# near/near-light-client

Measured on AMD Instinct MI355X. Metric: Sync/Verify proofs/sec at 1/2/4/8 MI355X + achieved HBM GB/s vs roofline, higher is better.
Workload: dtype u64 (Goldilocks field, integer)

## Files before the change

near-light-client_amd/csrc/gl32.hpp:

```cpp
#pragma once
#include "gl.hpp"
#include "poseidon_blocks.inc"

namespace gl32 {

struct F {
    uint32_t lo, hi;
};

__device__ __forceinline__ F from_u64(uint64_t x) { return F{(uint32_t)x, (uint32_t)(x >> 32)}; }
__device__ __forceinline__ uint64_t to_u64(F x) { return ((uint64_t)x.hi << 32) | x.lo; }

__device__ __forceinline__ F add_w2_eps(uint64_t base, uint32_t w2) {
    uint64_t r;
    uint32_t t;
    asm("v_mad_u64_u32 %[r], vcc, %[w2], -1, %[base]\n\t"
        "v_cndmask_b32_e64 %[t], 0, -1, vcc\n\t"
        "v_mad_u64_u32 %[r], vcc, %[t], 1, %[r]"
        : [r] "=&v"(r), [t] "=&v"(t)
        : [w2] "v"(w2), [base] "v"(base)
        : "vcc");
    return from_u64(r);
}

__device__ __forceinline__ F reduce128(uint32_t w0, uint32_t w1, uint32_t w2, uint32_t w3) {
    uint32_t r0, r1, t0;
    asm("v_sub_co_u32 %[r0], vcc, %[w0], %[w3]\n\t"
        "v_subbrev_co_u32 %[r1], vcc, 0, %[w1], vcc\n\t"
        "v_cndmask_b32_e64 %[t0], 0, -1, vcc\n\t"
        "v_sub_co_u32 %[r0], vcc, %[r0], %[t0]\n\t"
        "v_subbrev_co_u32 %[r1], vcc, 0, %[r1], vcc"
        : [r0] "=&v"(r0), [r1] "=&v"(r1), [t0] "=&v"(t0)
        : [w0] "v"(w0), [w1] "v"(w1), [w3] "v"(w3)
        : "vcc");
    return add_w2_eps(((uint64_t)r1 << 32) | r0, w2);
}

__device__ __forceinline__ uint64_t mad_u64_one(uint32_t a, uint64_t c);

__device__ __forceinline__ F mul(F a, F b) {
#ifdef NLX_GL32_MUL_CARRY_CHAINS
    uint64_t t = (uint64_t)a.lo * b.lo;
    uint64_t m = (uint64_t)a.lo * b.hi;
    uint64_t x = (uint64_t)a.hi * b.hi;
    uint64_t mid;
    uint32_t x1;
    asm("v_mad_u64_u32 %[mid], vcc, %[ah], %[bl], %[m]\n\t"
        "v_addc_co_u32 %[x1], vcc, 0, %[xh], vcc"
        : [mid] "=&v"(mid), [x1] "=v"(x1)
        : [ah] "v"(a.hi), [bl] "v"(b.lo), [m] "v"(m), [xh] "v"((uint32_t)(x >> 32))
        : "vcc");
    uint32_t r0, r1, w1, w2, w3, t0;
    asm("v_add_co_u32 %[w1], vcc, %[th], %[m0]\n\t"
        "v_addc_co_u32 %[w2], vcc, %[x0], %[m1], vcc\n\t"
        "v_addc_co_u32 %[w3], vcc, 0, %[x1], vcc\n\t"
        "v_sub_co_u32 %[r0], vcc, %[w0], %[w3]\n\t"
        "v_subbrev_co_u32 %[r1], vcc, 0, %[w1], vcc\n\t"
        "v_cndmask_b32_e64 %[t0], 0, -1, vcc\n\t"
        "v_sub_co_u32 %[r0], vcc, %[r0], %[t0]\n\t"
        "v_subbrev_co_u32 %[r1], vcc, 0, %[r1], vcc"
        : [r0] "=&v"(r0), [r1] "=&v"(r1), [w1] "=&v"(w1), [w2] "=&v"(w2), [w3] "=&v"(w3), [t0] "=&v"(t0)
        : [w0] "v"((uint32_t)t), [th] "v"((uint32_t)(t >> 32)), [m0] "v"((uint32_t)mid), [x0] "v"((uint32_t)x),
          [m1] "v"((uint32_t)(mid >> 32)), [x1] "v"(x1)
        : "vcc");
    return add_w2_eps(((uint64_t)r1 << 32) | r0, w2);
#else
    const uint64_t p0 = (uint64_t)a.lo * b.lo;
    const uint64_t p1 = (uint64_t)a.lo * b.hi + (p0 >> 32);
    const uint64_t p2 = (uint64_t)a.hi * b.lo + (uint32_t)p1;
    uint64_t p3 = (uint64_t)a.hi * b.hi + (p1 >> 32);
    p3 = mad_u64_one((uint32_t)(p2 >> 32), p3);
    return reduce128((uint32_t)p0, (uint32_t)p2, (uint32_t)p3, (uint32_t)(p3 >> 32));
#endif
}

__device__ __forceinline__ F add_const(F a, uint64_t c) {
    F r;
    uint32_t t;
    asm("v_add_co_u32 %[r0], vcc, %[a0], %[c0]\n\t"
        "v_addc_co_u32 %[r1], vcc, %[a1], %[c1], vcc\n\t"
        "v_cndmask_b32_e64 %[t], 0, -1, vcc\n\t"
        "v_add_co_u32 %[r0], vcc, %[r0], %[t]\n\t"
        "v_addc_co_u32 %[r1], vcc, 0, %[r1], vcc"
        : [r0] "=&v"(r.lo), [r1] "=&v"(r.hi), [t] "=&v"(t)
        : [a0] "v"(a.lo), [a1] "v"(a.hi), [c0] "s"((uint32_t)c), [c1] "v"((uint32_t)(c >> 32))
        : "vcc");
    return r;
}

__device__ __forceinline__ F add_const_v(F a, uint64_t c) {
    F r;
    uint32_t t;
    asm("v_add_co_u32 %[r0], vcc, %[a0], %[c0]\n\t"
        "v_addc_co_u32 %[r1], vcc, %[a1], %[c1], vcc\n\t"
        "v_cndmask_b32_e64 %[t], 0, -1, vcc\n\t"
        "v_add_co_u32 %[r0], vcc, %[r0], %[t]\n\t"
        "v_addc_co_u32 %[r1], vcc, 0, %[r1], vcc"
        : [r0] "=&v"(r.lo), [r1] "=&v"(r.hi), [t] "=&v"(t)
        : [a0] "v"(a.lo), [a1] "v"(a.hi), [c0] "v"((uint32_t)c), [c1] "v"((uint32_t)(c >> 32))
        : "vcc");
    return r;
}

__device__ __forceinline__ F sbox7(F x) {
    F x2 = mul(x, x);
    F x4 = mul(x2, x2);
    F x3 = mul(x, x2);
    return mul(x3, x4);
}

__device__ __forceinline__ F fold_acc(uint64_t al, uint64_t ah) {
    uint64_t t;
    asm("v_mad_u64_u32 %[t], vcc, %[ah1], -1, %[al]" : [t] "=&v"(t) : [ah1] "v"((uint32_t)(ah >> 32)), [al] "v"(al) : "vcc");
    uint32_t r1, m;
    asm("v_add_co_u32 %[r1], vcc, %[t1], %[ah0]\n\t"
        "v_cndmask_b32_e64 %[m], 0, -1, vcc"
        : [r1] "=v"(r1), [m] "=v"(m)
        : [t1] "v"((uint32_t)(t >> 32)), [ah0] "v"((uint32_t)ah)
        : "vcc");
    uint64_t r;
    asm("v_mad_u64_u32 %[r], vcc, %[m], 1, %[base]" : [r] "=&v"(r) : [m] "v"(m), [base] "v"(((uint64_t)r1 << 32) | (uint32_t)t) : "vcc");
    return from_u64(r);
}

__device__ __forceinline__ void mds_layer(F (&s)[12], const uint64_t* __restrict__ rc_next = nullptr) {
    constexpr uint32_t C[12] = {17, 15, 41, 16, 2, 28, 13, 13, 39, 18, 34, 20};
    F o[12];
#pragma unroll
    for (int r = 0; r < 12; r++) {
        uint64_t al = 0, ah = 0;
        if (rc_next) {
            const uint64_t c = rc_next[r];
            al = (uint32_t)c;
            ah = c >> 32;
        }
#pragma unroll
        for (int i = 0; i < 12; i++) {
            al += (uint64_t)s[(i + r) % 12].lo * C[i];
            ah += (uint64_t)s[(i + r) % 12].hi * C[i];
        }
        if (r == 0) {
            al += (uint64_t)s[0].lo * 8u;
            ah += (uint64_t)s[0].hi * 8u;
        }
        o[r] = fold_acc(al, ah);
    }
#pragma unroll
    for (int i = 0; i < 12; i++) s[i] = o[i];
}


typedef int i32x4_t __attribute__((ext_vector_type(4)));
typedef int i32x16_t __attribute__((ext_vector_type(16)));

__device__ __forceinline__ void keep_whole(const i32x16_t& d) { asm volatile("" : : "v"(d)); }

__device__ __forceinline__ i32x4_t mds_a_fragment(uint32_t lane = threadIdx.x & 63) {
    constexpr int C[12] = {17, 15, 41, 16, 2, 28, 13, 13, 39, 18, 34, 20};
    const uint32_t rho = lane & 31, h = lane >> 5;
    const uint32_t g = (rho >> 2) & 1, r = (rho & 3) + 4 * (rho >> 3);
    uint32_t w[4] = {0, 0, 0, 0};
    if (h == g && rho < 24) {
#pragma unroll
        for (int j = 0; j < 12; j++) {
            uint32_t m = 0;
#pragma unroll
            for (int rr = 0; rr < 12; rr++)
                if ((uint32_t)rr == r) m = (uint32_t)C[(j - rr + 12) % 12] + ((rr == 0 && j == 0) ? 8u : 0u);
            w[j >> 2] |= m << (8 * (j & 3));
        }
        w[3] = r == 0 ? 0x00F88080u : 0x00008080u;
    }
    i32x4_t a;
    a.x = (int)w[0]; a.y = (int)w[1]; a.z = (int)w[2]; a.w = (int)w[3];
    return a;
}
constexpr uint32_t MDS_B_BIAS_SLOTS = 0x00808080u;

__device__ __forceinline__ void transpose_bytes4(uint32_t x0, uint32_t x1, uint32_t x2, uint32_t x3, uint32_t (&p)[4]) {
    const uint32_t t01l = __builtin_amdgcn_perm(x1, x0, 0x05010400u), t01h = __builtin_amdgcn_perm(x1, x0, 0x07030602u);
    const uint32_t t23l = __builtin_amdgcn_perm(x3, x2, 0x05010400u), t23h = __builtin_amdgcn_perm(x3, x2, 0x07030602u);
    p[0] = __builtin_amdgcn_perm(t23l, t01l, 0x05040100u);
    p[1] = __builtin_amdgcn_perm(t23l, t01l, 0x07060302u);
    p[2] = __builtin_amdgcn_perm(t23h, t01h, 0x05040100u);
    p[3] = __builtin_amdgcn_perm(t23h, t01h, 0x07060302u);
}
__device__ __forceinline__ uint64_t mad_u64(uint32_t a, uint32_t b, uint64_t c) {
    uint64_t r, sink;
    asm("v_mad_u64_u32 %0, %1, %2, %3, %4" : "=v"(r), "=s"(sink) : "v"(a), "v"(b), "v"(c));
    return r;
}
__device__ __forceinline__ uint64_t mad_u64_sc(uint32_t a, uint32_t b, uint64_t c_uniform) {
    uint64_t r, sink;
    asm("v_mad_u64_u32 %0, %1, %2, %3, %4" : "=v"(r), "=s"(sink) : "v"(a), "v"(b), "s"(c_uniform));
    return r;
}
__device__ __forceinline__ uint64_t mad_u64_one(uint32_t a, uint64_t c) {
    uint64_t r, sink;
    asm("v_mad_u64_u32 %0, %1, %2, 1, %3" : "=v"(r), "=s"(sink) : "v"(a), "v"(c));
    return r;
}
__device__ __forceinline__ F fold_pair(uint64_t t, uint32_t yh, uint32_t k16) {
    uint64_t z, u, sink, sink2;
    asm("v_mad_u64_u32 %0, %1, %2, %3, 0" : "=v"(z), "=s"(sink) : "v"(yh), "v"(k16));
    asm("v_mad_u64_u32 %0, %1, %2, -1, %3" : "=v"(u), "=s"(sink2) : "v"((uint32_t)(z >> 32)), "v"(t));
    uint32_t r1, m;
    asm("v_add_co_u32 %0, vcc, %2, %3\n\t"
        "v_cndmask_b32_e64 %1, 0, -1, vcc"
        : "=v"(r1), "=v"(m)
        : "v"((uint32_t)(u >> 32)), "v"((uint32_t)z)
        : "vcc");
    return from_u64(mad_u64_one(m, ((uint64_t)r1 << 32) | (uint32_t)u));
}

template <int RC>
__device__ __forceinline__ void mds_layer_mfma(F (&s)[12], const i32x4_t a, const uint64_t* __restrict__ rcb) {
    uint32_t k16 = 65536u, bw = MDS_B_BIAS_SLOTS;
    asm("" : "+v"(k16));
    asm("" : "+v"(bw));
    i32x16_t zero;
#pragma unroll
    for (int i = 0; i < 16; i++) zero[i] = 0;
    uint32_t x[2][12], y[2][12];
#pragma unroll
    for (int half = 0; half < 2; half++) {
        uint32_t pl[4][3];
#pragma unroll
        for (int q = 0; q < 3; q++) {
            uint32_t p[4];
            if (half == 0)
                transpose_bytes4(s[4 * q].lo ^ 0x80808080u, s[4 * q + 1].lo ^ 0x80808080u, s[4 * q + 2].lo ^ 0x80808080u,
                                 s[4 * q + 3].lo ^ 0x80808080u, p);
            else
                transpose_bytes4(s[4 * q].hi ^ 0x80808080u, s[4 * q + 1].hi ^ 0x80808080u, s[4 * q + 2].hi ^ 0x80808080u,
                                 s[4 * q + 3].hi ^ 0x80808080u, p);
#pragma unroll
            for (int b = 0; b < 4; b++) pl[b][q] = p[b];
        }
        i32x16_t d[4];
#pragma unroll
        for (int b = 0; b < 4; b++) {
            i32x4_t bf;
            bf.x = (int)pl[b][0]; bf.y = (int)pl[b][1]; bf.z = (int)pl[b][2]; bf.w = (int)bw;
            d[b] = __builtin_amdgcn_mfma_i32_32x32x32_i8(a, bf, zero, 0, 0, 0);
        }
#pragma unroll
        for (int b = 0; b < 4; b++) keep_whole(d[b]);
#pragma unroll
        for (int r = 0; r < 12; r++) {
            x[half][r] = ((uint32_t)d[1][r] << 8) + (uint32_t)d[0][r];
            y[half][r] = ((uint32_t)d[3][r] << 8) + (uint32_t)d[2][r];
        }
        __builtin_amdgcn_sched_barrier(0);
    }
#pragma unroll
    for (int r = 0; r < 12; r++) {
        if (RC == 2 || (RC == 1 && r == 0)) {
            const uint64_t al = mad_u64_one(x[0][r], mad_u64_sc(y[0][r], k16, rcb[r]));
            const uint64_t ah = mad_u64_one(x[1][r], mad_u64_sc(y[1][r], k16, rcb[12 + r]));
            s[r] = fold_acc(al, ah);
        } else {
            const uint64_t t = mad_u64(y[0][r], k16, ((uint64_t)x[1][r] << 32) | x[0][r]);
            s[r] = fold_pair(t, y[1][r], k16);
        }
    }
}

struct BlockOperands {
    i32x4_t a[3];
    i32x16_t seed;
};

template <int G>
__device__ __forceinline__ uint64_t mad_u64_imm(uint32_t a, uint64_t c) {
    uint64_t r, sink;
    asm("v_mad_u64_u32 %0, %1, %2, %3, %4" : "=v"(r), "=s"(sink) : "v"(a), "n"(G), "v"(c));
    return r;
}
__device__ __forceinline__ F fold_pair_x(uint64_t t, uint32_t yh, uint32_t x2, uint32_t k16) {
    uint64_t z, u, sink, sink2;
    asm("v_mad_u64_u32 %0, %1, %2, %3, 0" : "=v"(z), "=s"(sink) : "v"(yh), "v"(k16));
    const uint32_t e = (uint32_t)(z >> 32) + x2;
    asm("v_mad_u64_u32 %0, %1, %2, -1, %3" : "=v"(u), "=s"(sink2) : "v"(e), "v"(t));
    uint32_t r1, m;
    asm("v_add_co_u32 %0, vcc, %2, %3\n\t"
        "v_cndmask_b32_e64 %1, 0, -1, vcc"
        : "=v"(r1), "=v"(m)
        : "v"((uint32_t)(u >> 32)), "v"((uint32_t)z)
        : "vcc");
    return from_u64(mad_u64_one(m, ((uint64_t)r1 << 32) | (uint32_t)u));
}
__device__ __forceinline__ uint64_t mad_u64_sm(uint32_t a, uint32_t m_uniform, uint64_t c) {
    uint64_t r, sink;
    asm("v_mad_u64_u32 %0, %1, %2, %3, %4" : "=v"(r), "=s"(sink) : "v"(a), "s"(m_uniform), "v"(c));
    return r;
}
template <typename RHO>
__device__ __forceinline__ void dot12(const F (&z)[12], const RHO& rho, uint64_t klo, uint64_t khi, uint64_t& al, uint64_t& ah) {
    al = klo;
    ah = khi;
#pragma unroll
    for (int j = 0; j < 12; j++) {
        al = mad_u64_sm(z[j].lo, rho.v[j], al);
        ah = mad_u64_sm(z[j].hi, rho.v[j], ah);
    }
}
struct BlockRho1 { static constexpr uint32_t v[12] = NLX_POSEIDON_BLOCK_RHO1_INIT; };
struct BlockRho2 { static constexpr uint32_t v[12] = NLX_POSEIDON_BLOCK_RHO2_INIT; };

struct BlockSboxes {
    __device__ __forceinline__ F first(F s0) const { return sbox7(s0); }
    __device__ __forceinline__ F inner(int, F w) const { return sbox7(w); }
    __device__ __forceinline__ void before_matrix_pass() const {}
};

template <int GAMMA21, class Sboxes = BlockSboxes>
__device__ __forceinline__ void partial_block3(F (&s)[12], const BlockOperands& op, const uint64_t* __restrict__ kap,
                                               Sboxes sb = Sboxes{}) {
    uint32_t k16 = 65536u;
    asm("" : "+v"(k16));
    s[0] = sb.first(s[0]);
    uint64_t al, ah;
    dot12(s, BlockRho1{}, kap[2], kap[3], al, ah);
    const F u1 = sb.inner(1, fold_acc(al, ah));
    dot12(s, BlockRho2{}, kap[4], kap[5], al, ah);
    al = mad_u64_imm<GAMMA21>(u1.lo, al);
    ah = mad_u64_imm<GAMMA21>(u1.hi, ah);
    const F u2 = sb.inner(2, fold_acc(al, ah));
    sb.before_matrix_pass();
    uint32_t pl[8][3];
#pragma unroll
    for (int half = 0; half < 2; half++)
#pragma unroll
        for (int q = 0; q < 3; q++) {
            uint32_t p[4];
            if (half == 0)
                transpose_bytes4(s[4 * q].lo ^ 0x80808080u, s[4 * q + 1].lo ^ 0x80808080u, s[4 * q + 2].lo ^ 0x80808080u,
                                 s[4 * q + 3].lo ^ 0x80808080u, p);
            else
                transpose_bytes4(s[4 * q].hi ^ 0x80808080u, s[4 * q + 1].hi ^ 0x80808080u, s[4 * q + 2].hi ^ 0x80808080u,
                                 s[4 * q + 3].hi ^ 0x80808080u, p);
#pragma unroll
            for (int b = 0; b < 4; b++) pl[4 * half + b][q] = p[b];
        }
    uint32_t w3[8];
    {
        const uint32_t a1l = u1.lo ^ 0x80808080u, a1h = u1.hi ^ 0x80808080u, a2l = u2.lo ^ 0x80808080u, a2h = u2.hi ^ 0x80808080u;
        w3[0] = __builtin_amdgcn_perm(a2l, a1l, 0x00000400u); w3[1] = __builtin_amdgcn_perm(a2l, a1l, 0x00000501u);
        w3[2] = __builtin_amdgcn_perm(a2l, a1l, 0x00000602u); w3[3] = __builtin_amdgcn_perm(a2l, a1l, 0x00000703u);
        w3[4] = __builtin_amdgcn_perm(a2h, a1h, 0x00000400u); w3[5] = __builtin_amdgcn_perm(a2h, a1h, 0x00000501u);
        w3[6] = __builtin_amdgcn_perm(a2h, a1h, 0x00000602u); w3[7] = __builtin_amdgcn_perm(a2h, a1h, 0x00000703u);
    }
    uint32_t x0[12], y0[12], y1[12];
    uint64_t tt[12];
    uint64_t ah0 = 0;
    auto chain = [&](int q) {
        i32x16_t d = op.seed;
#pragma unroll
        for (int p = 0; p < 3; p++)
            if (q - p >= 0 && q - p <= 7) {
                i32x4_t bf;
                bf.x = (int)pl[q - p][0]; bf.y = (int)pl[q - p][1]; bf.z = (int)pl[q - p][2]; bf.w = (int)w3[q - p];
                d = __builtin_amdgcn_mfma_i32_32x32x32_i8(op.a[p], bf, d, 0, 0, 0);
            }
        return d;
    };
#pragma unroll
    for (int pr = 0; pr < 5; pr++) {
        i32x16_t d[2];
        d[0] = chain(2 * pr);
        d[1] = chain(2 * pr + 1);
        keep_whole(d[0]);
        keep_whole(d[1]);
#pragma unroll
        for (int r = 0; r < 12; r++) {
            uint32_t x = ((uint32_t)d[1][r] << 8) + (uint32_t)d[0][r];
            asm("" : "+v"(x));
            if (pr == 0) x0[r] = x;
            if (pr == 1) {
                y0[r] = x;
                if (r == 0) tt[0] = mad_u64_one(x0[0], mad_u64_sc(x, k16, kap[0]));
            }
            if (pr == 2) {
                if (r == 0) ah0 = x;
                else tt[r] = mad_u64(y0[r], k16, ((uint64_t)x << 32) | x0[r]);
            }
            if (pr == 3) {
                y1[r] = x;
                if (r == 0) ah0 = mad_u64_one((uint32_t)ah0, mad_u64_sc(x, k16, kap[1]));
            }
            if (pr == 4) {
                if (r == 0) s[0] = fold_acc(tt[0], ah0 + ((uint64_t)x << 32));
                else s[r] = fold_pair_x(tt[r], y1[r], x, k16);
            }
        }
#ifndef NLX_PB_NO_BARRIER
        __builtin_amdgcn_sched_barrier(0);
#endif
    }
}

}
```

near-light-client_amd/csrc/hash_kernels.hip:

```cpp
#include <hip/hip_runtime.h>
#include "poseidon.hpp"
#include "launch.hpp"

namespace nlx {

__global__ __launch_bounds__(256, 4) void k_permute_batch(uint64_t* __restrict__ states, size_t n) {
    const size_t t_raw = (size_t)blockIdx.x * blockDim.x + threadIdx.x;
    const bool live = t_raw < n;
    const size_t t = live ? t_raw : n - 1;
    uint64_t s[12];
    const ulonglong2* src = reinterpret_cast<const ulonglong2*>(states + t * 12);
#pragma unroll
    for (int i = 0; i < 6; i++) {
        ulonglong2 v = src[i];
        s[2 * i] = v.x;
        s[2 * i + 1] = v.y;
    }
    poseidon::permute(s);
    if (!live) return;
    ulonglong2* dst = reinterpret_cast<ulonglong2*>(states + t * 12);
#pragma unroll
    for (int i = 0; i < 6; i++) dst[i] = make_ulonglong2(s[2 * i], s[2 * i + 1]);
}

__device__ __forceinline__ void store_digest(uint64_t* __restrict__ out, size_t idx, const uint64_t (&s)[12]) {
    ulonglong2* dst = reinterpret_cast<ulonglong2*>(out + idx * 4);
    dst[0] = make_ulonglong2(gl::canon(s[0]), gl::canon(s[1]));
    dst[1] = make_ulonglong2(gl::canon(s[2]), gl::canon(s[3]));
}

__global__ __launch_bounds__(256, 4) void k_hash_leaves_rowmajor(const uint64_t* __restrict__ rows, uint32_t row_len,
                                                              size_t n_rows, uint64_t* __restrict__ digests) {
    const size_t row_raw = (size_t)blockIdx.x * blockDim.x + threadIdx.x;
    const bool live = row_raw < n_rows;
    const size_t row = live ? row_raw : n_rows - 1;
    uint64_t s[12];
#pragma unroll
    for (int i = 0; i < 12; i++) s[i] = 0;
    const uint64_t* p = rows + row * (size_t)row_len;
    if (row_len <= 4) {
        for (uint32_t c = 0; c < row_len; c++) {
            uint64_t v = p[c];
            if (c == 0) s[0] = v; else if (c == 1) s[1] = v; else if (c == 2) s[2] = v; else s[3] = v;
        }
        if (live) store_digest(digests, row, s);
        return;
    }
#pragma unroll 1
    for (uint32_t c = 0; c < row_len; c += 8) {
        const uint32_t rem = row_len - c;
#pragma unroll
        for (int j = 0; j < 8; j++)
            if ((uint32_t)j < rem) s[j] = p[c + j];
        poseidon::permute_loose(s);
    }
    if (live) store_digest(digests, row, s);
}

__global__ __launch_bounds__(256, 4) void k_merkle_level(const uint64_t* __restrict__ children,
                                                      uint64_t* __restrict__ parents, size_t n_parents, size_t tree_words) {
    children += (size_t)blockIdx.y * tree_words;
    parents += (size_t)blockIdx.y * tree_words;
    const size_t i_raw = (size_t)blockIdx.x * blockDim.x + threadIdx.x;
    const bool live = i_raw < n_parents;
    const size_t i = live ? i_raw : n_parents - 1;
    const ulonglong2* src = reinterpret_cast<const ulonglong2*>(children + i * 8);
    uint64_t s[12];
#pragma unroll
    for (int k = 0; k < 4; k++) {
        ulonglong2 v = src[k];
        s[2 * k] = v.x;
        s[2 * k + 1] = v.y;
    }
    s[8] = s[9] = s[10] = s[11] = 0;
    poseidon::permute_loose(s);
    if (live) store_digest(parents, i, s);
}

constexpr size_t MERKLE_WIDE_MAX_PARENTS = (size_t)1 << 13;
constexpr unsigned MERKLE_FUSED_MAX_LEVELS = 6;
void launch_merkle_fused(hipStream_t st, const uint64_t* children, size_t n_children, unsigned levels, uint32_t n_trees, size_t tree_words);

void launch_permute_batch(hipStream_t st, uint64_t* d_states, size_t n) {
    if (!n) return;
    hipLaunchKernelGGL(k_permute_batch, dim3((unsigned)((n + 255) / 256)), dim3(256), 0, st, d_states, n);
}

void launch_hash_leaves_rowmajor(hipStream_t st, const uint64_t* d_rows, uint32_t row_len, size_t n_rows,
                                 uint64_t* d_digests) {
    if (!n_rows) return;
    hipLaunchKernelGGL(k_hash_leaves_rowmajor, dim3((unsigned)((n_rows + 255) / 256)), dim3(256), 0, st, d_rows,
                       row_len, n_rows, d_digests);
}

const uint64_t* launch_merkle_levels(hipStream_t st, uint64_t* d_digests, size_t n_leaves, unsigned cap_height, uint32_t n_trees, size_t tree_words) {
    size_t cap = (size_t)1 << cap_height;
    uint64_t* cur = d_digests;
    size_t lvl = n_leaves;
    while (lvl > cap) {
        uint64_t* nxt = cur + lvl * 4;
        size_t half = lvl >> 1;
        if (half * n_trees <= MERKLE_WIDE_MAX_PARENTS) {
            unsigned K = 0;
            while (K < MERKLE_FUSED_MAX_LEVELS && (lvl >> K) > cap) K++;
            launch_merkle_fused(st, cur, lvl, K, n_trees, tree_words);
            for (unsigned s = 0; s < K; s++) {
                cur += lvl * 4;
                lvl >>= 1;
            }
            continue;
        }
        hipLaunchKernelGGL(k_merkle_level, dim3((unsigned)((half + 255) / 256), n_trees), dim3(256), 0, st, cur, nxt, half, tree_words);
        cur = nxt;
        lvl = half;
    }
    return cur;
}

}

namespace nlx {

constexpr size_t HASH_LEAVES_WIDE_MAX_ROWS = (size_t)1 << 13;

__global__ __launch_bounds__(256, 4) void k_hash_lde_leaves(const uint64_t* __restrict__ lde, size_t col_stride,
                                                         uint32_t n_cols, unsigned log_n, unsigned rate_bits,
                                                         uint64_t* __restrict__ digests, uint32_t batch_cols, size_t tree_words) {
    if (batch_cols) {
        const uint32_t c0 = blockIdx.y * batch_cols;
        lde += (size_t)c0 * col_stride;
        n_cols = n_cols - c0 < batch_cols ? n_cols - c0 : batch_cols;
        digests += (size_t)blockIdx.y * tree_words;
    }
    const size_t pos_raw = (size_t)blockIdx.x * blockDim.x + threadIdx.x;
    const bool live = (pos_raw >> (log_n + rate_bits)) == 0;
    const size_t pos = live ? pos_raw : ((size_t)1 << (log_n + rate_bits)) - 1;
    uint64_t s[12];
#pragma unroll
    for (int i = 0; i < 12; i++) s[i] = 0;
    const uint64_t* p = lde + pos;
    const uint32_t r = (uint32_t)(pos >> log_n), k = (uint32_t)(pos & (((size_t)1 << log_n) - 1));
    const size_t leaf = ((size_t)gl::bitrev32(r, rate_bits) << log_n) + gl::bitrev32(k, log_n);
    if (n_cols <= 4) {
        for (uint32_t c = 0; c < n_cols; c++) {
            uint64_t v = p[(size_t)c * col_stride];
            if (c == 0) s[0] = v; else if (c == 1) s[1] = v; else if (c == 2) s[2] = v; else s[3] = v;
        }
        if (live) store_digest(digests, leaf, s);
        return;
    }
#pragma unroll 1
    for (uint32_t c = 0; c < n_cols; c += 8) {
        const uint32_t rem = n_cols - c;
#pragma unroll
        for (int j = 0; j < 8; j++)
            if ((uint32_t)j < rem) s[j] = p[(size_t)(c + j) * col_stride];
        poseidon::permute_loose(s);
    }
    if (live) store_digest(digests, leaf, s);
}

void launch_hash_lde_leaves_wide(hipStream_t st, const uint64_t* d_lde, size_t col_stride, uint32_t n_cols, unsigned log_n,
                                 unsigned rate_bits, uint64_t* d_digests, uint32_t batch_cols, size_t tree_words);

__global__ __launch_bounds__(256, 4) void k_hash_lde_groups(const uint64_t* __restrict__ lde, size_t col_stride, uint32_t n_cols,
                                                            uint32_t group, unsigned log_L, uint64_t* __restrict__ out) {
    const size_t pos_raw = (size_t)blockIdx.x * blockDim.x + threadIdx.x;
    const bool live = (pos_raw >> log_L) == 0;
    const size_t L = (size_t)1 << log_L, pos = live ? pos_raw : L - 1;
    const uint32_t g = blockIdx.y, c0 = g * group, c1 = c0 + group < n_cols ? c0 + group : n_cols;
    uint64_t s[12];
#pragma unroll
    for (int i = 0; i < 12; i++) s[i] = 0;
    const uint64_t* p = lde + pos;
#pragma unroll 1
    for (uint32_t c = c0; c < c1; c += 8) {
        const uint32_t rem = c1 - c;
#pragma unroll
        for (int j = 0; j < 8; j++)
            if ((uint32_t)j < rem) s[j] = p[(size_t)(c + j) * col_stride];
        poseidon::permute_loose(s);
    }
    if (!live) return;
#pragma unroll
    for (int j = 0; j < 4; j++) out[((size_t)(4 * g + j) << log_L) + pos] = gl::canon(s[j]);
}

void launch_hash_lde_leaves_grouped(hipStream_t st, const uint64_t* d_lde, size_t col_stride, uint32_t n_cols, uint32_t group,
                                    unsigned log_n, unsigned rate_bits, uint64_t* d_group_digests, uint64_t* d_digests) {
    const size_t rows = (size_t)1 << (log_n + rate_bits);
    const uint32_t K = (n_cols + group - 1) / group;
    hipLaunchKernelGGL(k_hash_lde_groups, dim3((unsigned)((rows + 255) / 256), K), dim3(256), 0, st, d_lde, col_stride, n_cols, group,
                       log_n + rate_bits, d_group_digests);
    launch_hash_lde_leaves(st, d_group_digests, rows, 4 * K, log_n, rate_bits, d_digests, 0, 0);
}

void launch_hash_lde_leaves(hipStream_t st, const uint64_t* d_lde, size_t col_stride, uint32_t n_cols,
                            unsigned log_n, unsigned rate_bits, uint64_t* d_digests, uint32_t batch_cols, size_t tree_words) {
    size_t rows = (size_t)1 << (log_n + rate_bits);
    const uint32_t n_batches = batch_cols ? (n_cols + batch_cols - 1) / batch_cols : 1;
    const uint32_t widest = batch_cols && batch_cols < n_cols ? batch_cols : n_cols;
    if (rows * n_batches <= HASH_LEAVES_WIDE_MAX_ROWS && widest > 16) {
        launch_hash_lde_leaves_wide(st, d_lde, col_stride, n_cols, log_n, rate_bits, d_digests, batch_cols, tree_words);
        return;
    }
    hipLaunchKernelGGL(k_hash_lde_leaves, dim3((unsigned)((rows + 255) / 256), n_batches), dim3(256), 0, st, d_lde, col_stride,
                       n_cols, log_n, rate_bits, d_digests, batch_cols, tree_words);
}

}

#include "poseidon_quad.hpp"

namespace nlx {

constexpr unsigned QUADS_PER_BLOCK = 16;

constexpr unsigned FUSED_QUADS = 32;

__global__ __launch_bounds__(FUSED_QUADS * 4) void k_merkle_fused(const uint64_t* __restrict__ children, uint64_t* __restrict__ parents0,
                                                                  size_t n_children, unsigned K, size_t tree_words) {
    children += (size_t)blockIdx.y * tree_words;
    parents0 += (size_t)blockIdx.y * tree_words;
    __shared__ uint64_t lv[2][FUSED_QUADS * 2 * 4];
    const uint32_t q = threadIdx.x & 3, g = threadIdx.x >> 2;
    const pquad::Mds mds = pquad::mds_table(q);
    const uint32_t n_own = 1u << K;
    for (uint32_t i = threadIdx.x; i < n_own * 4; i += FUSED_QUADS * 4) lv[0][i] = children[((size_t)blockIdx.x << K) * 4 + i];
    __syncthreads();
    uint64_t* outp = parents0;
    size_t level_total = n_children;
    for (unsigned s = 1; s <= K; s++) {
        const uint32_t own = n_own >> s;
        level_total >>= 1;
        const uint64_t* src = lv[(s - 1) & 1];
        uint64_t* dst = lv[s & 1];
        if (g < own) {
            gl32::F x[3] = {gl32::from_u64(src[g * 8 + q]), gl32::from_u64(src[g * 8 + 4 + q]), gl32::from_u64(0)};
            pquad::permute(x, q, mds);
            const uint64_t w = gl::canon(gl32::to_u64(x[0]));
            dst[g * 4 + q] = w;
            outp[((size_t)blockIdx.x * own + g) * 4 + q] = w;
        }
        __syncthreads();
        outp += level_total * 4;
    }
}

template <int ARITY_BITS>
__global__ __launch_bounds__(QUADS_PER_BLOCK * 4) void k_fri_leaves_wide(const uint64_t* __restrict__ values, unsigned log_n,
                                                                         unsigned rate_bits, uint64_t* __restrict__ digests) {
    constexpr int ARITY = 1 << ARITY_BITS;
    const unsigned log_np = log_n - ARITY_BITS;
    const uint32_t q = threadIdx.x & 3;
    const size_t n_leaves = (size_t)1 << (log_np + rate_bits);
    const size_t jp_raw = (size_t)blockIdx.x * QUADS_PER_BLOCK + (threadIdx.x >> 2);
    const bool live = jp_raw < n_leaves;
    const size_t jp = live ? jp_raw : n_leaves - 1;
    const size_t np = (size_t)1 << log_np, n = (size_t)1 << log_n;
    const uint32_t r = (uint32_t)(jp >> log_np), kp = (uint32_t)(jp & (np - 1));
    const pquad::Mds mds = pquad::mds_table(q);
    gl32::F x[3] = {gl32::from_u64(0), gl32::from_u64(0), gl32::from_u64(0)};
#pragma unroll 1
    for (int m0 = 0; m0 < ARITY; m0 += 4) {
#pragma unroll
        for (int h = 0; h < 2; h++) {
            const uint32_t j = q + 4 * h;
            const uint32_t mm = gl::bitrev32((uint32_t)m0 + (j >> 1), ARITY_BITS);
            x[h] = gl32::from_u64(values[2 * ((size_t)r * n + kp + (size_t)mm * np) + (j & 1)]);
        }
        pquad::permute(x, q, mds);
    }
    if (live) {
        const size_t leaf = ((size_t)gl::bitrev32(r, rate_bits) << log_np) + gl::bitrev32(kp, log_np);
        digests[leaf * 4 + q] = gl::canon(gl32::to_u64(x[0]));
    }
}

__global__ __launch_bounds__(QUADS_PER_BLOCK * 4) void k_hash_lde_leaves_wide(const uint64_t* __restrict__ lde, size_t col_stride, uint32_t n_cols,
                                                                              unsigned log_n, unsigned rate_bits, uint64_t* __restrict__ digests,
                                                                              uint32_t batch_cols, size_t tree_words) {
    if (batch_cols) {
        const uint32_t c0 = blockIdx.y * batch_cols;
        lde += (size_t)c0 * col_stride;
        n_cols = n_cols - c0 < batch_cols ? n_cols - c0 : batch_cols;
        digests += (size_t)blockIdx.y * tree_words;
    }
    const uint32_t q = threadIdx.x & 3;
    const size_t rows = (size_t)1 << (log_n + rate_bits);
    const size_t pos_raw = (size_t)blockIdx.x * QUADS_PER_BLOCK + (threadIdx.x >> 2);
    const bool live = pos_raw < rows;
    const size_t pos = live ? pos_raw : rows - 1;
    const uint64_t* p = lde + pos;
    gl32::F x[3] = {gl32::from_u64(0), gl32::from_u64(0), gl32::from_u64(0)};
    if (n_cols <= 4) {
        if (q < n_cols) x[0] = gl32::from_u64(p[(size_t)q * col_stride]);
    } else {
        const pquad::Mds mds = pquad::mds_table(q);
#pragma unroll 1
        for (uint32_t c = 0; c < n_cols; c += 8) {
            if (c + q < n_cols) x[0] = gl32::from_u64(p[(size_t)(c + q) * col_stride]);
            if (c + 4 + q < n_cols) x[1] = gl32::from_u64(p[(size_t)(c + 4 + q) * col_stride]);
            pquad::permute(x, q, mds);
        }
    }
    if (live) {
        const uint32_t r = (uint32_t)(pos >> log_n), k = (uint32_t)(pos & (((size_t)1 << log_n) - 1));
        const size_t leaf = ((size_t)gl::bitrev32(r, rate_bits) << log_n) + gl::bitrev32(k, log_n);
        digests[leaf * 4 + q] = gl::canon(gl32::to_u64(x[0]));
    }
}

void launch_hash_lde_leaves_wide(hipStream_t st, const uint64_t* d_lde, size_t col_stride, uint32_t n_cols, unsigned log_n,
                                 unsigned rate_bits, uint64_t* d_digests, uint32_t batch_cols, size_t tree_words) {
    const size_t rows = (size_t)1 << (log_n + rate_bits);
    const uint32_t n_batches = batch_cols ? (n_cols + batch_cols - 1) / batch_cols : 1;
    hipLaunchKernelGGL(k_hash_lde_leaves_wide, dim3((unsigned)((rows + QUADS_PER_BLOCK - 1) / QUADS_PER_BLOCK), n_batches), dim3(QUADS_PER_BLOCK * 4), 0,
                       st, d_lde, col_stride, n_cols, log_n, rate_bits, d_digests, batch_cols, tree_words);
}

void launch_fri_leaves_wide(hipStream_t st, const uint64_t* d_values, unsigned log_n, unsigned rate_bits,
                            unsigned arity_bits, uint64_t* d_digests) {
    const size_t leaves = (size_t)1 << (log_n - arity_bits + rate_bits);
    const unsigned blocks = (unsigned)((leaves + QUADS_PER_BLOCK - 1) / QUADS_PER_BLOCK);
    const dim3 threads(QUADS_PER_BLOCK * 4);
    if (arity_bits == 4) hipLaunchKernelGGL(k_fri_leaves_wide<4>, dim3(blocks), threads, 0, st, d_values, log_n, rate_bits, d_digests);
    else if (arity_bits == 3) hipLaunchKernelGGL(k_fri_leaves_wide<3>, dim3(blocks), threads, 0, st, d_values, log_n, rate_bits, d_digests);
    else if (arity_bits == 2) hipLaunchKernelGGL(k_fri_leaves_wide<2>, dim3(blocks), threads, 0, st, d_values, log_n, rate_bits, d_digests);
}

void launch_merkle_fused(hipStream_t st, const uint64_t* children, size_t n_children, unsigned levels, uint32_t n_trees, size_t tree_words) {
    hipLaunchKernelGGL(k_merkle_fused, dim3((unsigned)(n_children >> levels), n_trees), dim3(FUSED_QUADS * 4), 0, st, children,
                       const_cast<uint64_t*>(children) + n_children * 4, n_children, levels, tree_words);
}

}
```

near-light-client_amd/csrc/poseidon.hpp:

```cpp
#pragma once
#include "gl.hpp"
#if defined(__HIP__)
#include "gl32.hpp"
#endif
#include "poseidon_constants.inc"

namespace poseidon {

constexpr int WIDTH = 12;
constexpr int RATE = 8;
constexpr int N_ROUNDS = 30;
constexpr int HALF_FULL = 4;
constexpr int N_PARTIAL = 22;

#if defined(__HIP__)
__constant__ static const uint64_t RC_DEV[360] = NLX_POSEIDON_ROUND_CONSTANTS_INIT;
__constant__ static const uint64_t LAYER_RCB_DEV[31 * 24] = NLX_POSEIDON_LAYER_RCB_INIT;
__constant__ static const uint32_t BLOCK_FRAGMENTS_DEV[NLX_POSEIDON_BLOCK_K * 64 * 4] = NLX_POSEIDON_BLOCK_FRAGMENTS_INIT;
__constant__ static const uint32_t BLOCK_SEED_DEV[16] = NLX_POSEIDON_BLOCK_SEED_INIT;
__constant__ static const uint64_t BLOCK_KAPPA_DEV[NLX_POSEIDON_N_BLOCKS * 2 * NLX_POSEIDON_BLOCK_K] = NLX_POSEIDON_BLOCK_KAPPA_INIT;
static_assert(NLX_POSEIDON_BLOCK_K == 3 && NLX_POSEIDON_BLOCK_DMAX < (1 << 20), "gl32::partial_block3 is written for these");

__device__ __forceinline__ gl32::BlockOperands block_operands(uint32_t lane = threadIdx.x & 63) {
    gl32::BlockOperands op;
#pragma unroll
    for (int p = 0; p < 3; p++) {
        const uint32_t* f = BLOCK_FRAGMENTS_DEV + (p * 64 + lane) * 4;
        op.a[p].x = (int)f[0]; op.a[p].y = (int)f[1]; op.a[p].z = (int)f[2]; op.a[p].w = (int)f[3];
    }
    const uint32_t zero = lane >> 6;
#pragma unroll
    for (int i = 0; i < 16; i++) op.seed[i] = (int)(BLOCK_SEED_DEV[i] + zero);
    return op;
}
#endif
static const uint64_t RC_HOST[360] = NLX_POSEIDON_ROUND_CONSTANTS_INIT;

GL_HD const uint64_t* rc_table() {
#if defined(__HIP_DEVICE_COMPILE__)
    return RC_DEV;
#else
    return RC_HOST;
#endif
}

GL_HD uint64_t sbox7(uint64_t x) {
    uint64_t x2 = gl::mul_loose(x, x);
    uint64_t x4 = gl::mul_loose(x2, x2);
    uint64_t x3 = gl::mul_loose(x, x2);
    return gl::mul_loose(x3, x4);
}

GL_HD uint64_t mds_fold(uint64_t al, uint64_t ah) {
    uint64_t l = al + (ah << 32);
    uint64_t h = (ah >> 32) + (l < al ? 1u : 0u);
    uint64_t t1 = (h << 32) - h;
    uint64_t res = l + t1;
    if (res < t1) res += gl::EPS;
    return res;
}
GL_HD void mds_layer(uint64_t (&s)[12]) {
    constexpr uint32_t C[12] = {17, 15, 41, 16, 2, 28, 13, 13, 39, 18, 34, 20};
    uint32_t lo[12], hi[12];
#pragma unroll
    for (int i = 0; i < 12; i++) {
        lo[i] = (uint32_t)s[i];
        hi[i] = (uint32_t)(s[i] >> 32);
    }
#pragma unroll
    for (int r = 0; r < 12; r++) {
        uint64_t al = 0, ah = 0;
#pragma unroll
        for (int i = 0; i < 12; i++) {
            al += (uint64_t)lo[(i + r) % 12] * C[i];
            ah += (uint64_t)hi[(i + r) % 12] * C[i];
        }
        if (r == 0) {
            al += (uint64_t)lo[0] * 8u;
            ah += (uint64_t)hi[0] * 8u;
        }
        s[r] = mds_fold(al, ah);
    }
}

GL_HD void permute_loose(uint64_t (&s)[12]) {
    const uint64_t* rc = rc_table();
#if defined(__HIP_DEVICE_COMPILE__)
#if defined(NLX_DEBUG)
    if (__builtin_amdgcn_read_exec() != ~0ull) __builtin_trap();
#endif
    const uint64_t* rcb = LAYER_RCB_DEV;
    const gl32::i32x4_t a = gl32::mds_a_fragment();
    const gl32::BlockOperands op = block_operands();
    gl32::F t[12];
#pragma unroll
    for (int i = 0; i < 12; i++) t[i] = gl32::add_const(gl32::from_u64(s[i]), rc[i]);
#pragma unroll 1
    for (int r = 0; r < HALF_FULL; r++) {
#pragma unroll
        for (int i = 0; i < 12; i++) t[i] = gl32::sbox7(t[i]);
        gl32::mds_layer_mfma<2>(t, a, rcb + (r + 1) * 24);
    }
#pragma unroll 1
    for (int b = 0; b < NLX_POSEIDON_N_BLOCKS; b++)
        gl32::partial_block3<NLX_POSEIDON_BLOCK_GAMMA21>(t, op, BLOCK_KAPPA_DEV + b * 6);
    t[0] = gl32::sbox7(t[0]);
    gl32::mds_layer_mfma<2>(t, a, rcb + (HALF_FULL + N_PARTIAL) * 24);
#pragma unroll 1
    for (int r = HALF_FULL + N_PARTIAL; r < N_ROUNDS - 1; r++) {
#pragma unroll
        for (int i = 0; i < 12; i++) t[i] = gl32::sbox7(t[i]);
        gl32::mds_layer_mfma<2>(t, a, rcb + (r + 1) * 24);
    }
#pragma unroll
    for (int i = 0; i < 12; i++) t[i] = gl32::sbox7(t[i]);
    gl32::mds_layer_mfma<0>(t, a, rcb);
#pragma unroll
    for (int i = 0; i < 12; i++) s[i] = gl32::to_u64(t[i]);
#else
#pragma unroll 1
    for (int r = 0; r < HALF_FULL; r++) {
        for (int i = 0; i < 12; i++) s[i] = sbox7(gl::add_loose(s[i], rc[r * 12 + i]));
        mds_layer(s);
    }
    for (int r = HALF_FULL; r < HALF_FULL + N_PARTIAL; r++) {
        for (int i = 0; i < 12; i++) s[i] = gl::add_loose(s[i], rc[r * 12 + i]);
        s[0] = sbox7(s[0]);
        mds_layer(s);
    }
    for (int r = HALF_FULL + N_PARTIAL; r < N_ROUNDS; r++) {
        for (int i = 0; i < 12; i++) s[i] = sbox7(gl::add_loose(s[i], rc[r * 12 + i]));
        mds_layer(s);
    }
#endif
}

GL_HD void permute(uint64_t (&s)[12]) {
    permute_loose(s);
#pragma unroll
    for (int i = 0; i < 12; i++) s[i] = gl::canon(s[i]);
}

}
```

Before: 23.44.

## Add sponge-specialized Poseidon permutation skipping unused final MDS outputs and zero-capacity sbox

```diff
diff --git a/near-light-client_amd/csrc/gl32.hpp b/near-light-client_amd/csrc/gl32.hpp
--- a/near-light-client_amd/csrc/gl32.hpp
+++ b/near-light-client_amd/csrc/gl32.hpp
@@ -88,6 +88,20 @@
     return r;
 }
 
+__device__ __forceinline__ F add_const_s(F a, uint64_t c_uniform) {
+    uint64_t t, sink;
+    asm("v_mad_u64_u32 %0, %1, %2, 1, %3" : "=v"(t), "=s"(sink) : "v"(a.lo), "s"(c_uniform));
+    uint32_t r1, m;
+    asm("v_add_co_u32 %0, vcc, %2, %3\n\t"
+        "v_cndmask_b32_e64 %1, 0, -1, vcc"
+        : "=v"(r1), "=v"(m)
+        : "v"((uint32_t)(t >> 32)), "v"(a.hi)
+        : "vcc");
+    uint64_t r, sink2;
+    asm("v_mad_u64_u32 %0, %1, %2, 1, %3" : "=v"(r), "=s"(sink2) : "v"(m), "v"(((uint64_t)r1 << 32) | (uint32_t)t));
+    return from_u64(r);
+}
+
 __device__ __forceinline__ F add_const_v(F a, uint64_t c) {
     F r;
     uint32_t t;
@@ -264,6 +278,69 @@
             s[r] = fold_pair(t, y[1][r], k16);
         }
     }
+}
+
+constexpr uint32_t KEEP_DIGEST = 1u, KEEP_RATE_TOP = 2u, KEEP_CAPACITY = 4u, KEEP_ALL = 7u;
+template <bool SEED_CAP>
+__device__ __forceinline__ void mds_layer_mfma_keep(F (&s)[12], const i32x4_t a, const uint64_t* __restrict__ rc0, uint32_t keep) {
+    uint32_t k16 = 65536u, bw = MDS_B_BIAS_SLOTS;
+    asm("" : "+v"(k16));
+    asm("" : "+v"(bw));
+    i32x16_t zero;
+#pragma unroll
+    for (int i = 0; i < 16; i++) zero[i] = 0;
+    uint32_t x[2][12], y[2][12];
+#pragma unroll
+    for (int half = 0; half < 2; half++) {
+        uint32_t pl[4][3];
+#pragma unroll
+        for (int q = 0; q < 3; q++) {
+            uint32_t p[4];
+            if (half == 0)
+                transpose_bytes4(s[4 * q].lo ^ 0x80808080u, s[4 * q + 1].lo ^ 0x80808080u, s[4 * q + 2].lo ^ 0x80808080u,
+                                 s[4 * q + 3].lo ^ 0x80808080u, p);
+            else
+                transpose_bytes4(s[4 * q].hi ^ 0x80808080u, s[4 * q + 1].hi ^ 0x80808080u, s[4 * q + 2].hi ^ 0x80808080u,
+                                 s[4 * q + 3].hi ^ 0x80808080u, p);
+#pragma unroll
+            for (int b = 0; b < 4; b++) pl[b][q] = p[b];
+        }
+        i32x16_t d[4];
+#pragma unroll
+        for (int b = 0; b < 4; b++) {
+            i32x4_t bf;
+            bf.x = (int)pl[b][0]; bf.y = (int)pl[b][1]; bf.z = (int)pl[b][2]; bf.w = (int)bw;
+            d[b] = __builtin_amdgcn_mfma_i32_32x32x32_i8(a, bf, zero, 0, 0, 0);
+        }
+#pragma unroll
+        for (int b = 0; b < 4; b++) keep_whole(d[b]);
+#pragma unroll
+        for (int g = 0; g < 3; g++)
+            if (keep & (1u << g)) {
+#pragma unroll
+                for (int r = 4 * g; r < 4 * g + 4; r++) {
+                    x[half][r] = ((uint32_t)d[1][r] << 8) + (uint32_t)d[0][r];
+                    y[half][r] = ((uint32_t)d[3][r] << 8) + (uint32_t)d[2][r];
+                }
+            }
+        __builtin_amdgcn_sched_barrier(0);
+    }
+#pragma unroll
+    for (int g = 0; g < 3; g++)
+        if (keep & (1u << g)) {
+#pragma unroll
+            for (int r = 4 * g; r < 4 * g + 4; r++) {
+                if (SEED_CAP && g == 2) {
+                    const uint64_t c = rc0[r];
+                    const uint64_t al = mad_u64_one(x[0][r], mad_u64_sc(y[0][r], k16, (uint32_t)c));
+                    const uint64_t ah = mad_u64_one(x[1][r], mad_u64_sc(y[1][r], k16, c >> 32));
+                    s[r] = fold_acc(al, ah);
+                } else {
+                    const uint64_t t = mad_u64(y[0][r], k16, ((uint64_t)x[1][r] << 32) | x[0][r]);
+                    s[r] = fold_pair(t, y[1][r], k16);
+                }
+            }
+        }
 }
 
 struct BlockOperands {
diff --git a/near-light-client_amd/csrc/hash_kernels.hip b/near-light-client_amd/csrc/hash_kernels.hip
--- a/near-light-client_amd/csrc/hash_kernels.hip
+++ b/near-light-client_amd/csrc/hash_kernels.hip
@@ -52,7 +52,7 @@
 #pragma unroll
         for (int j = 0; j < 8; j++)
             if ((uint32_t)j < rem) s[j] = p[c + j];
-        poseidon::permute_loose(s);
+        poseidon::permute_sponge(s, poseidon::sponge_keep(rem), c == 0);
     }
     if (live) store_digest(digests, row, s);
 }
@@ -73,7 +73,7 @@
         s[2 * k + 1] = v.y;
     }
     s[8] = s[9] = s[10] = s[11] = 0;
-    poseidon::permute_loose(s);
+    poseidon::permute_sponge(s, gl32::KEEP_DIGEST, true);
     if (live) store_digest(parents, i, s);
 }
 
@@ -155,7 +155,7 @@
 #pragma unroll
         for (int j = 0; j < 8; j++)
             if ((uint32_t)j < rem) s[j] = p[(size_t)(c + j) * col_stride];
-        poseidon::permute_loose(s);
+        poseidon::permute_sponge(s, poseidon::sponge_keep(rem), c == 0);
     }
     if (live) store_digest(digests, leaf, s);
 }
@@ -179,7 +179,7 @@
 #pragma unroll
         for (int j = 0; j < 8; j++)
             if ((uint32_t)j < rem) s[j] = p[(size_t)(c + j) * col_stride];
-        poseidon::permute_loose(s);
+        poseidon::permute_sponge(s, poseidon::sponge_keep(rem), c == c0);
     }
     if (!live) return;
 #pragma unroll
diff --git a/near-light-client_amd/csrc/poseidon.hpp b/near-light-client_amd/csrc/poseidon.hpp
--- a/near-light-client_amd/csrc/poseidon.hpp
+++ b/near-light-client_amd/csrc/poseidon.hpp
@@ -34,7 +34,7 @@
     return op;
 }
 #endif
-static const uint64_t RC_HOST[360] = NLX_POSEIDON_ROUND_CONSTANTS_INIT;
+static constexpr uint64_t RC_HOST[360] = NLX_POSEIDON_ROUND_CONSTANTS_INIT;
 
 GL_HD const uint64_t* rc_table() {
 #if defined(__HIP_DEVICE_COMPILE__)
@@ -83,22 +83,35 @@
     }
 }
 
-GL_HD void permute_loose(uint64_t (&s)[12]) {
+#if defined(__HIP__)
+constexpr uint64_t ce_mul(uint64_t a, uint64_t b) { return (uint64_t)((unsigned __int128)a * b % gl::P); }
+constexpr uint64_t ce_sbox7(uint64_t x) { return ce_mul(ce_mul(ce_mul(x, x), x), ce_mul(ce_mul(x, x), ce_mul(x, x))); }
+constexpr uint64_t SBOX_RC0_CAP[4] = {ce_sbox7(RC_HOST[8]), ce_sbox7(RC_HOST[9]), ce_sbox7(RC_HOST[10]), ce_sbox7(RC_HOST[11])};
+
+__device__ __forceinline__ uint32_t sponge_keep(uint32_t rem) {
+    return rem <= (uint32_t)RATE ? gl32::KEEP_DIGEST : rem < 2u * RATE ? gl32::KEEP_ALL : gl32::KEEP_CAPACITY;
+}
+
+template <bool SPONGE>
+__device__ __forceinline__ void permute_rounds(gl32::F (&t)[12], uint32_t keep, bool zero_capacity) {
     const uint64_t* rc = rc_table();
-#if defined(__HIP_DEVICE_COMPILE__)
 #if defined(NLX_DEBUG)
-    if (__builtin_amdgcn_read_exec() != ~0ull) __builtin_trap();
+    if (__builtin_amdgcn_read_exec() != ~0ull || (SPONGE && !keep)) __builtin_trap();
 #endif
     const uint64_t* rcb = LAYER_RCB_DEV;
     const gl32::i32x4_t a = gl32::mds_a_fragment();
     const gl32::BlockOperands op = block_operands();
-    gl32::F t[12];
-#pragma unroll
-    for (int i = 0; i < 12; i++) t[i] = gl32::add_const(gl32::from_u64(s[i]), rc[i]);
 #pragma unroll 1
     for (int r = 0; r < HALF_FULL; r++) {
 #pragma unroll
-        for (int i = 0; i < 12; i++) t[i] = gl32::sbox7(t[i]);
+        for (int i = 0; i < RATE; i++) t[i] = gl32::sbox7(t[i]);
+        if (SPONGE && zero_capacity && r == 0) {
+#pragma unroll
+            for (int i = 0; i < 4; i++) t[RATE + i] = gl32::from_u64(SBOX_RC0_CAP[i]);
+        } else {
+#pragma unroll
+            for (int i = RATE; i < 12; i++) t[i] = gl32::sbox7(t[i]);
+        }
         gl32::mds_layer_mfma<2>(t, a, rcb + (r + 1) * 24);
     }
 #pragma unroll 1
@@ -114,7 +127,18 @@
     }
 #pragma unroll
     for (int i = 0; i < 12; i++) t[i] = gl32::sbox7(t[i]);
-    gl32::mds_layer_mfma<0>(t, a, rcb);
+    if (SPONGE) gl32::mds_layer_mfma_keep<true>(t, a, rc, keep);
+    else gl32::mds_layer_mfma<0>(t, a, rcb);
+}
+#endif
+
+GL_HD void permute_loose(uint64_t (&s)[12]) {
+    const uint64_t* rc = rc_table();
+#if defined(__HIP_DEVICE_COMPILE__)
+    gl32::F t[12];
+#pragma unroll
+    for (int i = 0; i < 12; i++) t[i] = gl32::add_const(gl32::from_u64(s[i]), rc[i]);
+    permute_rounds<false>(t, gl32::KEEP_ALL, false);
 #pragma unroll
     for (int i = 0; i < 12; i++) s[i] = gl32::to_u64(t[i]);
 #else
@@ -135,6 +159,24 @@
 #endif
 }
 
+#if defined(__HIP__)
+__device__ __forceinline__ void permute_sponge(uint64_t (&s)[12], uint32_t keep, bool zero_capacity) {
+#ifdef NLX_POSEIDON_SPONGE_FULL
+    permute_loose(s);
+#else
+    const uint64_t* rc = rc_table();
+    gl32::F t[12];
+#pragma unroll
+    for (int i = 0; i < RATE; i++) t[i] = gl32::add_const_s(gl32::from_u64(s[i]), rc[i]);
+#pragma unroll
+    for (int i = RATE; i < 12; i++) t[i] = gl32::from_u64(s[i]);
+    permute_rounds<true>(t, keep, zero_capacity);
+#pragma unroll
+    for (int i = 0; i < 12; i++) s[i] = gl32::to_u64(t[i]);
+#endif
+}
+#endif
+
 GL_HD void permute(uint64_t (&s)[12]) {
     permute_loose(s);
 #pragma unroll
```

Result: no change. 23.49 (median of 5 runs) (+0.2%).
